# stojicnnnn/3DVision

Measured on AMD Instinct MI355X. Metric: RANSAC hyps/s + ICP iters/s @ 200k-pt clouds, higher is better.
Workload: dtype f32

## Files before the change

3dvision_amd/__init__.py:

```python
import ctypes as C
import os
import sys
import threading
from dataclasses import dataclass, field
from typing import Optional

import numpy as np

_HERE = os.path.dirname(os.path.abspath(__file__))
STUDY_BUILD = os.environ.get("TDV_LIB_VARIANT") == "study"
LIB_PATH = os.path.join(_HERE, "lib3dvision_hip_study.so" if STUDY_BUILD else "lib3dvision_hip.so")

TDV_MASK_THRESHOLD10 = 0
TDV_MASK_NONZERO = 1
TDV_MASK_LABEL_BASE = 256
TDV_VOXEL_ORDER_FIRST = 0
TDV_VOXEL_ORDER_REFERENCE = 1
TIMER_ICP_NN, TIMER_RANSAC_SCORE, TIMER_FEATURE_MATCH, TIMER_KNN, TIMER_RADIUS, TIMER_DEPTH, TIMER_VOXEL, TIMER_FM_INDEX = range(8)
DEPTH_BATCH_MASK_PASSES = 1

ABI_SYMBOLS = [
    "tdv_device_count", "tdv_ctx_create", "tdv_ctx_set_stream", "tdv_ctx_set_icp_search", "tdv_ctx_set_icp_accumulation", "tdv_ctx_last_icp_search", "tdv_ctx_last_batch_lanes", "tdv_ctx_last_voxel_grouping", "tdv_ctx_last_voxel_batch_redone", "tdv_ctx_last_feature_match_path", "tdv_ctx_workspace_bytes", "tdv_ctx_workspace_fill", "tdv_ctx_set_ransac_score", "tdv_ctx_set_ransac_leaf_order", "tdv_ctx_last_ransac_rescore", "tdv_ctx_last_ransac_scored", "tdv_ctx_last_ransac_bound", "tdv_ctx_get_stream", "tdv_ctx_synchronize",
    "tdv_ctx_destroy", "tdv_status_string", "tdv_last_error", "tdv_version", "tdv_timing_enable", "tdv_timing_read",
    "tdv_depth_preprocess", "tdv_deproject", "tdv_depth_to_cloud", "tdv_voxel_downsample", "tdv_estimate_normals",
    "tdv_compute_fpfh", "tdv_feature_match", "tdv_ransac", "tdv_icp", "tdv_icp_correspondences",
    "tdv_icp_dev", "tdv_ransac_dev", "tdv_feature_match_dev", "tdv_estimate_normals_dev", "tdv_compute_fpfh_dev", "tdv_normals_fpfh_dev", "tdv_radix_sort_pairs_dev",
    "tdv_depth_to_cloud_dev", "tdv_voxel_downsample_dev", "tdv_sample_triples", "tdv_sample_triples_batch", "tdv_pose_compose",
    "tdv_register_batch_dev", "tdv_prepare_model_dev", "tdv_bilateral_filter", "tdv_filter_duplicates", "tdv_ransac_score_unit", "tdv_ransac_score_unit_block", "tdv_ransac_score_unit_chunks", "tdv_ransac_batch_size", "tdv_voxel_rules", "tdv_load_ply_ascii", "tdv_load_mask_png", "tdv_load_masks_from_dir",
    "tdv_depth_to_cloud_batch_dev", "tdv_broadcast_model", "tdv_gather_results", "tdv_mask_resize_nearest", "tdv_mask_resize_nearest_dev", "tdv_voxel_downsample_batch_dev", "tdv_voxel_downsample_batch_pinhole_dev",
    "tdv_icp_batch_dev", "tdv_refine_batch_dev", "tdv_ctx_set_icp_loss", "tdv_ctx_get_icp_loss",
    "tdv_gicp", "tdv_gicp_dev", "tdv_gicp_batch_dev",
    "tdv_color_gradients", "tdv_color_gradients_dev", "tdv_colored_icp", "tdv_colored_icp_dev", "tdv_colored_icp_batch_dev",
    "tdv_fgr_default_params", "tdv_fgr", "tdv_fgr_dev", "tdv_fgr_correspondences",
    "tdv_plane_default_params", "tdv_segment_planes", "tdv_segment_planes_dev",
    "tdv_cluster_default_params", "tdv_cluster_dbscan", "tdv_cluster_dbscan_dev",
    "tdv_remove_statistical_outlier", "tdv_remove_statistical_outlier_dev", "tdv_remove_radius_outlier", "tdv_remove_radius_outlier_dev",
    "tdv_iss_default_params", "tdv_iss_keypoints", "tdv_iss_keypoints_dev",
# ... 526 lines not shown
        if kind != "l2" and scale is None:
            raise ValueError("the %s loss needs a scale" % kind)
        _check(self._h, lib().tdv_ctx_set_icp_loss(self._h, self.ICP_LOSS[kind], C.c_float(0.0 if scale is None else float(scale))),
               "tdv_ctx_set_icp_loss")

    def icp_loss(self):
        k = C.c_int(); sc = C.c_float()
        _check(self._h, lib().tdv_ctx_get_icp_loss(self._h, C.byref(k), C.byref(sc)), "tdv_ctx_get_icp_loss")
        return {v: n for n, v in self.ICP_LOSS.items()}[k.value], float(sc.value)

    def set_ransac_score(self, mode):
        _check(self._h, lib().tdv_ctx_set_ransac_score(self._h, {"fast": 0, "exact": 1, "matrix": 2}[mode]), "tdv_ctx_set_ransac_score")

    def set_ransac_leaf_order(self, mode):
        _check(self._h, lib().tdv_ctx_set_ransac_leaf_order(self._h, {"auto": 0, "morton": 1, "classes": 2}[mode]), "tdv_ctx_set_ransac_leaf_order")

    def last_ransac_rescore(self):
        return float(lib().tdv_ctx_last_ransac_rescore(self._h))

    def last_ransac_scored(self):
        return float(lib().tdv_ctx_last_ransac_scored(self._h))

    def last_ransac_bound(self):
        out = (C.c_longlong * 4)()
        lib().tdv_ctx_last_ransac_bound(self._h, out)
        return tuple(int(v) for v in out)

    def last_feature_match_path(self):
        return {0: "none", 1: "scan", 2: "leaf_major", 3: "walk"}[int(lib().tdv_ctx_last_feature_match_path(self._h))]

# ... 1255 lines not shown
```

3dvision_amd/csrc/batch.hip:

```cpp
#include "tdv_internal.hpp"
#include <algorithm>
#include <functional>
#include <thread>
#include <cstdio>
#include <cstdlib>
#include <cstring>
#include <vector>

namespace tdv {

__global__ void k_globalise(const int* __restrict__ local, const int* __restrict__ voff, int n_inst, int total, int* __restrict__ out) {
    const int P = blockIdx.x * blockDim.x + threadIdx.x;
    if (P >= total) return;
    int a = 0, z = n_inst;
    while (z - a > 1) { const int m = (a + z) >> 1; if (voff[m] <= P) a = m; else z = m; }
    out[P] = local[P] + voff[a];
}

__global__ void k_gather_i32(const int* __restrict__ in, const int* __restrict__ idx, int n, int* __restrict__ out) {
    const int p = blockIdx.x * blockDim.x + threadIdx.x;
    if (p < n) out[p] = in[idx[p]];
}

namespace {
// ... 231 lines not shown
    const int L = (int)lane_ctx.size();
    ctx->last_batch_lanes = L;
    auto for_all_instances = [&](const std::function<int(tdv_ctx*, int)>& fn) -> int {
        if (L == 1) {
            int st = TDV_OK;
            for (int b = 0; b < n_instances && st == TDV_OK; ++b) st = fn(ctx, b);
            if (hipStreamSynchronize(ctx->stream) != hipSuccess && st == TDV_OK) st = TDV_ERR_LAUNCH;
            return st;
        }
        TDV_HIP(ctx, hipStreamSynchronize(ctx->stream));
        std::vector<int> status((size_t)L, TDV_OK);
        std::vector<std::thread> workers;
        for (int l = 1; l < L; ++l) {
            tdv_ctx* h = lane_ctx[l];
            h->timing = ctx->timing; h->icp_search = ctx->icp_search; h->icp_accumulate = ctx->icp_accumulate;
            h->icp_loss = ctx->icp_loss; h->icp_loss_scale = ctx->icp_loss_scale; h->ransac_score_mode = ctx->ransac_score_mode; h->ransac_leaf_order = ctx->ransac_leaf_order; h->err[0] = 0;
            workers.emplace_back([&, h, l]() {
                try {
                    if (hipSetDevice(h->device) != hipSuccess) { status[l] = TDV_ERR_NO_DEVICE; return; }
                    status[l] = ws_reset(h);
                    for (int b = l; b < n_instances && status[l] == TDV_OK; b += L) status[l] = fn(h, b);
                    if (hipStreamSynchronize(h->stream) != hipSuccess && status[l] == TDV_OK) status[l] = TDV_ERR_LAUNCH;
                } catch (...) {
                    std::snprintf(h->err, sizeof(h->err), "exception in a helper lane");
                    status[l] = TDV_ERR_INTERNAL;
                }
            });
        }
        try {
            for (int b = 0; b < n_instances && status[0] == TDV_OK; b += L) status[0] = fn(ctx, b);
        } catch (...) {
// ... 255 lines not shown
```

3dvision_amd/csrc/ctx.hip:

```cpp
#include "tdv_internal.hpp"
#include <cmath>
#include <cfloat>
#include <algorithm>
#include <cstring>
#include <vector>

namespace tdv {

int ws_reset(tdv_ctx* ctx) {
    if (ctx->blocks.size() > 1) {
        size_t total = 0;
        TDV_HIP(ctx, hipStreamSynchronize(ctx->stream));
        for (auto& b : ctx->blocks) { total += b.cap; (void)hipFree(b.p); }
        ctx->blocks.clear();
        total = align_up(total + total / 4, (size_t)1 << 20);
        char* p = nullptr;
        TDV_HIP(ctx, hipMalloc((void**)&p, total));
        ctx->blocks.push_back({p, total});
    }
    ctx->cur_block = 0; ctx->cur_off = 0; ctx->used_total = 0;
    return TDV_OK;
}

int ws_alloc_bytes(tdv_ctx* ctx, size_t bytes, void** out) {
// ... 290 lines not shown
    ctx->icp_search = mode;
    return TDV_OK;
}

int tdv_ctx_set_ransac_score(tdv_ctx* ctx, int mode) {
    if (!ctx || (mode != TDV_RANSAC_SCORE_FAST && mode != TDV_RANSAC_SCORE_EXACT && !(tdv::kStudyBuild && mode == TDV_RANSAC_SCORE_MATRIX))) return TDV_ERR_BAD_ARG;
    ctx->ransac_score_mode = mode;
    return TDV_OK;
}

int tdv_ctx_set_ransac_leaf_order(tdv_ctx* ctx, int mode) {
    if (!ctx || mode < TDV_RANSAC_LEAVES_AUTO || mode > TDV_RANSAC_LEAVES_CLASSES) return TDV_ERR_BAD_ARG;
    ctx->ransac_leaf_order = mode;
    return TDV_OK;
}

int tdv_ctx_set_fps_path(tdv_ctx* ctx, int mode) {
    if (!ctx || mode < TDV_FPS_AUTO || mode > TDV_FPS_GRID) return TDV_ERR_BAD_ARG;
    ctx->fps_path = mode;
    return TDV_OK;
}
int tdv_ctx_last_fps_path(tdv_ctx* ctx) { return ctx ? ctx->last_fps_path : 0; }

double tdv_ctx_last_ransac_rescore(tdv_ctx* ctx) { return ctx ? ctx->last_ransac_rescore : -1.0; }

double tdv_ctx_last_ransac_scored(tdv_ctx* ctx) { return ctx ? ctx->last_ransac_scored : 1.0; }
void tdv_ctx_last_ransac_bound(tdv_ctx* ctx, long long out[4]) { if (out) for (int e = 0; e < 4; ++e) out[e] = ctx ? ctx->last_ransac_bound[e] : 0; }

int tdv_ctx_last_icp_search(tdv_ctx* ctx) { return ctx ? ctx->last_icp_search : 0; }
int tdv_ctx_last_feature_match_path(tdv_ctx* ctx) { return ctx ? ctx->last_fm_path : 0; }
// ... 128 lines not shown
```

3dvision_amd/csrc/ransac.hip:

```cpp
#include "tdv_internal.hpp"
#include "host_wait.hpp"
#include "device_linalg.hpp"
#include "ransac_cut.hpp"
#include <cfloat>
#include <climits>
#include <cmath>
#include <cstddef>
#include <cstring>
#include <algorithm>
#include <type_traits>
#include <vector>

namespace tdv {

constexpr float kUnitRoundoff = 5.9604644775390625e-08f;
constexpr float kBandUnit = 16.f * kUnitRoundoff;
constexpr float kBandUnitMatrix = 24.f * kUnitRoundoff;

template <class I>
__device__ __forceinline__ float pair_record(const float* __restrict__ src, const float* __restrict__ tgt, const int* __restrict__ corr, I i, int nt,
                                             int* __restrict__ bad, float4& a, float4& b) {
    int c = corr[i];
    if ((unsigned)c >= (unsigned)nt) { *bad = 1; c = 0; }
    a = make_float4(src[3 * i], src[3 * i + 1], src[3 * i + 2], tgt[3 * c]);
// ... 949 lines not shown
    const unsigned long long m0 = __ballot(far), m1 = __ballot(near), m2 = __ballot(und);
    if (!(m0 | m1 | m2)) return 0;
    int at = 0;
    if (lane < 3) {
        const unsigned long long m = lane == 0 ? m0 : lane == 1 ? m1 : m2;
        int* const n = lane == 0 ? n_live : lane == 1 ? n_near : n_und;
        if (m) at = atomicAdd(n, __popcll(m));
    }
    const unsigned long long below = (1ull << lane) - 1ull;
    const int a0 = __shfl(at, 0, 64) + __popcll(m0 & below), a1 = __shfl(at, 1, 64) + __popcll(m1 & below), a2 = __shfl(at, 2, 64) + __popcll(m2 & below);
    if (far) live[a0] = h;
    if (near) nearl[a1] = h;
    if (und) undl[a2] = h;
    return a2;
}
template <int MODE>
__global__ __launch_bounds__(64 * RB_SPLIT)
void k_ransac_bound(const float* __restrict__ hyp, int h_pad, const TriView triples, int count, const float* __restrict__ leaves, int n_lpairs,
                    const unsigned* __restrict__ pmax, float sqrt_tau, float band_u, const int* __restrict__ state, int ns,
                    int* __restrict__ live, int* __restrict__ n_live, int* __restrict__ und, int* __restrict__ n_und,
                    int* __restrict__ acc, int* __restrict__ ticket, const ListJob lj) {
    const int lane = threadIdx.x & 63, wave = threadIdx.x >> 6;
    const int h = blockIdx.x * 64 + lane;
    __shared__ int s_ub[64];
    if (wave == 0) s_ub[lane] = 0;
    if (MODE == RB_COARSE && threadIdx.x == 0) ticket[blockIdx.x] = 0;
    const bool valid = h < count && triples.valid(h);
    const RbHyp o = rb_load(hyp, h_pad, h, valid, pmax, sqrt_tau, band_u, MODE == RB_COARSE ? 5.f : 3.f);
    const int best = state[0];
    const bool walk = rb_gate(best, ns);
    int fl = 0;
    if (wave == 0 && valid) fl = lj.flags[h];
    const int per = (n_lpairs + RB_SPLIT - 1) / RB_SPLIT, k0 = __builtin_amdgcn_readfirstlane(wave) * per, k1 = min(n_lpairs, k0 + per);
    const int ub = rb_walk(o.r, leaves, k0, k1, o.tb, best, !valid || !o.bounded || !walk);
    __syncthreads();
    if (ub) atomicAdd(&s_ub[lane], ub);
    __syncthreads();
    if (wave != 0) return;
    const int total = s_ub[lane];
    const bool gated = valid && (!o.bounded || !walk);
    const bool close = (fl & RB_CLOSE) != 0;
    const bool undecided = MODE == RB_COARSE && valid && !gated && !close && total > best;
    const bool is_live = gated || close || (MODE == RB_ONE && valid && total > best);
    const bool near = is_live && lj.near && (fl & RB_NEAR);
    const unsigned long long mc = __ballot(close);
    if (mc && lane == 0) atomicAdd(lj.n_close, __popcll(mc));
    const int slot = rb_append3(is_live && !near, near, undecided, lane, h, live, n_live, lj.near, lj.n_near, und, n_und);
    if (MODE == RB_COARSE && undecided) acc[slot] = 0;
}
// ... 132 lines not shown
    int plan[2][8];
    float best12[12];
    double out2[2];
    int sel[4];
    int rec[2][8];
    RansacFar far;
};
constexpr size_t kRansacReadBack = offsetof(RansacBlock, sel);
static_assert(std::is_trivially_copyable<RansacBlock>::value, "memset, copied back");
static_assert(offsetof(RansacBlock, rescored) % 8 == 0 && offsetof(RansacBlock, scored) == offsetof(RansacBlock, rescored) + 8, "the kernels index the two as one u64[2]");
static_assert(offsetof(RansacBlock, out2) % 8 == 0 && offsetof(RansacBlock, out2) + sizeof(double[2]) == kRansacReadBack, "the part read back is a prefix that ends with out2");
struct RansacLive { int n_live[2], n_und[2], n_near[2], n_close[2]; };
static_assert(offsetof(RansacLive, n_und) == offsetof(RansacLive, n_live) + 2 * sizeof(int) && offsetof(RansacLive, n_near) == offsetof(RansacLive, n_live) + 4 * sizeof(int) &&
              offsetof(RansacLive, n_close) == offsetof(RansacLive, n_live) + 6 * sizeof(int), "ransac_plan's n_live[2], n_live[4], n_live[6]");

struct RansacKnobs { bool score_fast, score_mfma, bailout, bound, one_level, leaf_classes, merge, record_copy, upload_inline, order, far, end_event, timer_events; int drop_permille, a_permille, u_cut_permille, fine_y, grown; float far_radius, live_radius; };
static RansacKnobs ransac_knobs(const tdv_ctx* ctx, bool traced, int max_iterations, int ns) {
    RansacKnobs k;
    static const bool score_exact_env = getenv("TDV_RANSAC_SCORE") && !strcmp(getenv("TDV_RANSAC_SCORE"), "exact");
    k.score_fast = !score_exact_env && ctx->ransac_score_mode != TDV_RANSAC_SCORE_EXACT;
    const bool score_mfma_env = study_env("TDV_RANSAC_SCORE") && !strcmp(study_env("TDV_RANSAC_SCORE"), "mfma");
    k.score_mfma = kStudyBuild && k.score_fast && (score_mfma_env || ctx->ransac_score_mode == TDV_RANSAC_SCORE_MATRIX);
    static const bool bailout_env_off = getenv("TDV_RANSAC_BAILOUT") && atoi(getenv("TDV_RANSAC_BAILOUT")) == 0;
    k.bailout = k.score_fast && !k.score_mfma && !traced && !bailout_env_off && max_iterations > 16384;
    k.merge = study_env("TDV_RANSAC_MERGE") && atoi(study_env("TDV_RANSAC_MERGE")) == 1;
    const bool bound_env_off = getenv("TDV_RANSAC_BOUND") && atoi(getenv("TDV_RANSAC_BOUND")) == 0;
    k.bound = k.bailout && !k.merge && !bound_env_off;
    const char* const order_env = getenv("TDV_RANSAC_ORDER");
    k.order = k.bailout && !k.merge && !(order_env && atoi(order_env) == 0);
    k.far = k.order && k.bound && !(order_env && atoi(order_env) == 1);
    k.far_radius = study_env("TDV_RANSAC_FAR_RADIUS") ? (float)atof(study_env("TDV_RANSAC_FAR_RADIUS")) : 4.f;
    k.a_permille = study_env("TDV_RANSAC_FAR_A_PERMILLE") ? atoi(study_env("TDV_RANSAC_FAR_A_PERMILLE")) : 110;
    k.u_cut_permille = study_env("TDV_RANSAC_FAR_UCUT_PERMILLE") ? atoi(study_env("TDV_RANSAC_FAR_UCUT_PERMILLE")) : 22;
    k.live_radius = study_env("TDV_RANSAC_LIVE_RADIUS") ? (float)atof(study_env("TDV_RANSAC_LIVE_RADIUS")) : 20.f;
    k.fine_y = study_env("TDV_RANSAC_FINE_Y") ? std::min(std::max(atoi(study_env("TDV_RANSAC_FINE_Y")), 1), kFineMaxRanges) : 0;
    k.grown = study_env("TDV_RANSAC_GROWN") ? (int)align_up((size_t)std::min(std::max(atoi(study_env("TDV_RANSAC_GROWN")), kRansacBatch), 4 * kRansacBatch), RS_HYP_PER_BLOCK) : kRansacGrown;
    k.leaf_classes = ctx->ransac_leaf_order == TDV_RANSAC_LEAVES_CLASSES || (ctx->ransac_leaf_order == TDV_RANSAC_LEAVES_AUTO && ns >= kRansacLeafClassesMin);
    if (study_env("TDV_RANSAC_LEAF_CLASSES")) k.leaf_classes = atoi(study_env("TDV_RANSAC_LEAF_CLASSES")) == 1;
    k.one_level = study_env("TDV_RANSAC_BOUND_LEVELS") && atoi(study_env("TDV_RANSAC_BOUND_LEVELS")) == 1;
    k.record_copy = study_env("TDV_RANSAC_RECORD") && !strcmp(study_env("TDV_RANSAC_RECORD"), "copy");
    k.end_event = traced || k.record_copy || (study_env("TDV_RANSAC_END") && !strcmp(study_env("TDV_RANSAC_END"), "event"));
    k.timer_events = study_env("TDV_RANSAC_TIMER") && !strcmp(study_env("TDV_RANSAC_TIMER"), "events");
    k.upload_inline = study_env("TDV_RANSAC_UPLOAD") && !strcmp(study_env("TDV_RANSAC_UPLOAD"), "inline");
    k.drop_permille = study_env("TDV_RANSAC_DROP_PERMILLE") ? atoi(study_env("TDV_RANSAC_DROP_PERMILLE")) : 50;
    return k;
}

struct RansacBuf {
    float* hyp; int* counts; void* tri; int* list;
    int *live, *und, *acc, *ticket;
    int *near, *list2, *ubf;
    int* flags;
    int* units;
    int *plan, *rec, *n_live, *n_und, *n_near;
    void* h_tri; int* h_cnt; volatile int* h_rec;
    hipEvent_t ev;
    int seq;
};
struct RansacBatch { int q, cnt, it0; bool bounded; };
struct RangeCut { int per, ranges; };
static RangeCut range_cut(int hb, int n_pchunks) {
    const int per = (n_pchunks + point_ranges(hb, n_pchunks) - 1) / point_ranges(hb, n_pchunks);
    return RangeCut{per, (n_pchunks + per - 1) / per};
}
static int hyp_blocks(int cnt) { return (int)(align_up((size_t)cnt, RS_HYP_PER_BLOCK) / RS_HYP_PER_BLOCK); }
static int score_grid(int hb, int ps) { return 8 * ((hb + 8 / RS_XCD_R - 1) / (8 / RS_XCD_R)) * ((ps + RS_XCD_R - 1) / RS_XCD_R); }
static int unit_grid(int cus) { return std::max(8, (2 * cus + 7) / 8 * 8); }
static int fine_grid(int cus) { return unit_grid(cus); }

struct RansacRun {
    tdv_ctx* ctx; hipStream_t s; RansacKnobs k;
    int ns, nt, max_iterations; float confidence; int* trace;
    float tau, sqrt_tau, band_u;
    int ns_pad, n_pchunks, batch, cap, h_pad, packed, rblocks, n_lpairs = 0, n_cpairs = 0, cus = 0;
    size_t tri_bytes;
    float *pq = nullptr, *pq2 = nullptr, *pq3 = nullptr, *leaves = nullptr, *cleaves = nullptr; double* slabs = nullptr;
    RansacBlock *d = nullptr, *h = nullptr; RansacLive* lv = nullptr;
    unsigned long long* leaf_keys = nullptr; unsigned* leaf_vals = nullptr; bool leaves_built = false;
    unsigned long long* ord_mask = nullptr; int* ord_cnt = nullptr; bool ordered = false;
    unsigned* enc = nullptr;
    RansacBuf buf[2] = {};
    unsigned long long *stamps = nullptr, *h_stamps = nullptr; int n_stamps = 0, stamps_used = 0;
    RansacBatch pending = {}; bool has_pending = false;
    double wave_chunks = 0.0;
    float best_fitness = 0.f; int best_iter = -1, best_inliers = 0, done_iters = 0; bool stop = false;

    TriView tri(const RansacBuf& B) const { return TriView{B.tri, packed}; }
    int setup(const float* d_src, const float* d_tgt, const int* d_corr) {
        ns_pad = (int)align_up((size_t)ns, (size_t)RS_PCH * 64);
        TDV_TRY(ws_alloc(ctx, (size_t)ns_pad * 8, &pq)); TDV_TRY(ws_alloc(ctx, 1, &d));
        TDV_HIP(ctx, hipMemsetAsync(d, 0, sizeof(RansacBlock), s));
        k_gather_pq<<<(ns_pad + 255) / 256, 256, 0, s>>>(d_src, d_tgt, d_corr, ns, ns_pad, nt, pq, &d->bad, &d->pmax);
        if (k.bound) TDV_TRY(leaf_alloc());
#ifdef TDV_STUDY
        if (k.score_mfma) TDV_TRY(mfma_pack(ctx, pq, ns, ns_pad, &pq3));
        else
// ... 21 lines not shown
                TDV_TRY(ws_alloc(ctx, (size_t)h_pad, &B.acc)); TDV_TRY(ws_alloc(ctx, (size_t)h_pad / 64, &B.ticket));
                TDV_TRY(ws_alloc(ctx, (size_t)h_pad, &B.flags));
            }
            TDV_TRY(ws_alloc(ctx, 1, &lv));
        }
        if (k.far) for (RansacBuf& B : buf) { TDV_TRY(ws_alloc(ctx, (size_t)h_pad, &B.near)); TDV_TRY(ws_alloc(ctx, (size_t)h_pad, &B.list2)); TDV_TRY(ws_alloc(ctx, (size_t)h_pad, &B.ubf)); }
        rblocks = (ns + 255) / 256; TDV_TRY(ws_alloc(ctx, (size_t)2 * rblocks, &slabs));
        if (ctx->timing && k.score_fast && !k.score_mfma && !k.timer_events) {
            n_stamps = 2 * n_batches + 1;
            TDV_TRY(ws_alloc(ctx, (size_t)2 * n_stamps, &stamps));
            TDV_HIP(ctx, hipMemsetAsync(stamps, 0xff, (size_t)n_stamps * 8, s));
            TDV_HIP(ctx, hipMemsetAsync(stamps + n_stamps, 0, (size_t)n_stamps * 8, s));
        }
        const size_t sz_blk = align_up(sizeof(RansacBlock), 64), sz_tri = align_up((size_t)cap * tri_bytes, 64), sz_cnt = trace ? align_up((size_t)cap * 4, 64) : 0;
        const size_t sz_grown = k.bailout ? 2 * align_up((size_t)k.grown * 16, 64) : 0;
        TDV_TRY(pin_reserve(ctx, sz_blk + std::max(2 * sz_tri, sz_grown) + 2 * sz_cnt + (size_t)n_stamps * 16));
        h = reinterpret_cast<RansacBlock*>(ctx->pin); h->bad = 0;
        h->rec[0][4] = h->rec[1][4] = 0;
        h_stamps = reinterpret_cast<unsigned long long*>(ctx->pin + sz_blk + 2 * sz_tri + 2 * sz_cnt);
        if (trace) TDV_HIP(ctx, hipMemcpyAsync(&h->bad, &d->bad, 4, hipMemcpyDeviceToHost, s));
        for (int q = 0; q < 2; ++q) {
            RansacBuf& B = buf[q];
            B.plan = d->plan[q]; B.rec = d->rec[q]; B.n_live = lv ? &lv->n_live[q] : nullptr; B.n_und = lv ? &lv->n_und[q] : nullptr; B.n_near = lv ? &lv->n_near[q] : nullptr;
            B.h_tri = ctx->pin + sz_blk + q * sz_tri; B.h_cnt = reinterpret_cast<int*>(ctx->pin + sz_blk + 2 * sz_tri + q * sz_cnt); B.h_rec = h->rec[q];
        }
        if (k.end_event) {
            buf[0].ev = event_acquire(ctx); buf[1].ev = event_acquire(ctx);
            if (!buf[0].ev || !buf[1].ev) { release_events(); return TDV_ERR_OOM; }
        }
        return TDV_OK;
    }
    ScoreStamp next_stamp() { if (!stamps || stamps_used >= n_stamps) return ScoreStamp{nullptr, nullptr}; const int e = stamps_used++; return ScoreStamp{stamps + e, stamps + n_stamps + e}; }
    int score_slot() const { return stamps ? -1 : TDV_TIMER_RANSAC_SCORE; }
    void launch_score(int grid, const ScoreJob& a, const ScoreJob& b, int g1) {
        const ScoreStamp st = next_stamp();
        if (st.t0) k_ransac_score_fast<true><<<grid, RS_BLOCK, 0, s>>>(a, b, g1, h_pad, pq2, n_pchunks, tau, &d->rescored, st);
        else k_ransac_score_fast<false><<<grid, RS_BLOCK, 0, s>>>(a, b, g1, h_pad, pq2, n_pchunks, tau, &d->rescored, st);
    }
    int batch_size(int it0) const { return k.bailout ? ransac_batch_size(it0, k.grown) : batch; }
// ... 10 lines not shown
    }
    int leaf_build() {
        const int n_leaves = (ns + RL_LEAF - 1) / RL_LEAF;
        unsigned long long* const keys = leaf_keys; unsigned* const vals = leaf_vals;
        TDV_HIP(ctx, hipMemsetAsync(leaves, 0, (size_t)n_lpairs * 32 * sizeof(float), s));
        TDV_HIP(ctx, hipMemsetAsync(cleaves, 0, (size_t)n_cpairs * 32 * sizeof(float), s));
        TDV_HIP(ctx, hipMemsetAsync(enc, 0xff, 24, s)); TDV_HIP(ctx, hipMemsetAsync(enc + 6, 0, 24, s));
        k_leaf_bounds<<<(ns + 255) / 256, 256, 0, s>>>(pq, ns, enc);
        k_leaf_keys<<<(ns + 255) / 256, 256, 0, s>>>(pq, ns, enc, k.leaf_classes && ordered ? ord_mask : nullptr, keys, vals);
        TDV_TRY(radix_sort_pairs_dev(ctx, keys, keys + ns, vals, vals + ns, (size_t)ns, RL_CLASS_BIT + (k.leaf_classes ? 1 : 0)));
        k_leaf_build<<<(n_leaves * RL_LEAF + 255) / 256, 256, 0, s>>>(pq, ns, vals + ns, leaves, cleaves);
        leaves_built = true;
        TDV_CHECK_LAUNCH(ctx); return TDV_OK;
    }

    int draw(TripleStream& idx, int q, int it0) {
        const int cnt = std::min(batch_size(it0), max_iterations - it0);
        if (packed) idx.next_batch_packed(cnt, static_cast<uint64_t*>(buf[q].h_tri));
        else idx.next_batch(cnt, static_cast<int*>(buf[q].h_tri));
        return cnt;
    }
    int hypotheses(const RansacBatch& b) {
        const RansacBuf& B = buf[b.q];
        if (k.upload_inline) TDV_HIP(ctx, hipMemcpyAsync(B.tri, B.h_tri, (size_t)b.cnt * tri_bytes, hipMemcpyHostToDevice, s));
        const PlanJob plan{d->state, k.bailout ? B.plan : nullptr, ns, n_pchunks, k.drop_permille, b.bounded ? B.n_live : nullptr, B.units, k.bailout ? unit_words(b.cnt) : 0,
                           k.far && b.bounded ? &d->far : nullptr, k.a_permille};
        const PreJob pre{b.bounded ? B.flags : nullptr, B.ubf, k.far ? &d->far : nullptr, enc, d->best12, k.live_radius, k.u_cut_permille};
        k_ransac_hypotheses<<<(slots(b.cnt) + 255) / 256, 256, 0, s>>>(pq, tri(B), k.upload_inline ? nullptr : B.h_tri, b.cnt, slots(b.cnt), h_pad, B.hyp, &d->pmax, sqrt_tau, B.counts, band_u, plan, pre);
        return TDV_OK;
    }
    int score_all(const RansacBatch& b) {
        const RansacBuf& B = buf[b.q]; const int hb = hyp_blocks(b.cnt);
        ScopedTimer tm(ctx, k.score_fast && !k.score_mfma ? score_slot() : TDV_TIMER_RANSAC_SCORE);
#ifdef TDV_STUDY
        if (k.score_mfma) wave_chunks += mfma_score(s, B.hyp, h_pad, pq3, ns, b.cnt, tau, B.counts, &d->rescored);
        else
#endif
        if (k.score_fast) {
            const ScoreJob ja{B.hyp, B.counts, nullptr, nullptr, hb, range_cut(hb, n_pchunks).ranges, nullptr, nullptr, nullptr};
            const int gA = score_grid(hb, ja.ps);
            launch_score(gA, ja, ja, gA);
            wave_chunks += (double)hb * (RS_BLOCK / 64) * (double)n_pchunks;
        } else {
            const RangeCut c = range_cut(h_pad / RS_HYP_PER_BLOCK, n_pchunks);
            k_ransac_score<<<dim3(hb, c.ranges), RS_BLOCK, 0, s>>>(B.hyp, h_pad, pq2, n_pchunks, c.per, tau, B.counts);
        }
        return TDV_OK;
    }
    void bound(const RansacBatch& b) {
        const RansacBuf& B = buf[b.q]; const int bgrid = (b.cnt + 63) / 64;
        const ListJob lj{B.flags, k.far ? B.near : nullptr, B.n_near, B.n_live + 6};
        if (k.one_level)
            k_ransac_bound<RB_ONE><<<bgrid, 64 * RB_SPLIT, 0, s>>>(B.hyp, h_pad, tri(B), b.cnt, leaves, n_lpairs, &d->pmax, sqrt_tau, band_u,
                                                                   d->state, ns, B.live, B.n_live, nullptr, nullptr, nullptr, nullptr, lj);
        else {
            k_ransac_bound<RB_COARSE><<<bgrid, 64 * RB_SPLIT, 0, s>>>(B.hyp, h_pad, tri(B), b.cnt, cleaves, n_cpairs, &d->pmax, sqrt_tau, band_u,
                                                                      d->state, ns, B.live, B.n_live, B.und, B.n_und, B.acc, B.ticket, lj);
            const FineJob fj{B.hyp, leaves, &d->pmax, d->state, B.und, B.n_und, B.live, B.n_live, B.acc, B.ticket, lj, h_pad, n_lpairs, k.fine_y, sqrt_tau, band_u};
            k_ransac_bound_fine<<<fine_grid(cus), 64 * RB_SPLIT, 0, s>>>(fj);
        }
    }
    void point_order() {
        RansacFar* const far = k.far ? &d->far : nullptr;
        k_order_flags<<<order_blocks(), RO_BLOCK, 0, s>>>(pq, ns, d->state, d->best12, tau, ord_mask, ord_cnt, far, std::max(tau, k.far_radius * k.far_radius * tau));
        k_order_scatter<<<order_blocks(), RO_BLOCK, 0, s>>>(pq, ns, ord_mask, ord_cnt, pq2, far);
        ordered = true;
    }
    ScoreJob job_a(const RansacBatch& b) const { return ScoreJob{buf[b.q].hyp, buf[b.q].counts, buf[b.q].plan, nullptr, hyp_blocks(b.cnt), range_cut(hyp_blocks(b.cnt), n_pchunks).ranges, nullptr, nullptr, nullptr}; }
    void phase1(const RansacBatch& b) {
        const RansacBuf& B = buf[b.q];
        const int hbw = slots(b.cnt) / RS_BLOCK;
        const ScoreJob ja = job_a(b), jl{B.hyp, B.counts, B.plan, B.live, hbw, 0, B.n_live, B.units, nullptr};
// ... 54 lines not shown
        std::snprintf(ctx->err, sizeof(ctx->err), "ransac: the stream ran dry and batch %d's record never came", B.seq);
        return TDV_ERR_LAUNCH;
    }
    int enqueue_merged(const RansacBatch& b) {
        if (has_pending) {
            const ScoreJob ja = job_a(b);
            TDV_TRY(phase2(pending, &ja, score_grid(ja.hb, ja.ps)));
            TDV_TRY(finish(pending, true));
        } else phase1(b);
        TDV_TRY(select(b));
        pending = b; has_pending = true;
        return TDV_OK;
    }
    int finish_pending() { has_pending = false; TDV_TRY(phase2(pending)); return finish(pending, true); }

    int enqueue(int q, int cnt, int it0) {
        const RansacBatch b{q, cnt, it0, k.bound && it0 != 0};
        if (k.order && it0 != 0 && !ordered) point_order();
        if (b.bounded && !leaves_built) TDV_TRY(leaf_build());
        TDV_TRY(hypotheses(b));
        if (!k.bailout) { TDV_TRY(score_all(b)); return finish(b, false); }
        if (k.merge) return enqueue_merged(b);
        if (b.bounded) bound(b);
        phase1(b);
        TDV_TRY(select(b));
        TDV_TRY(phase2(b));
        return finish(b, true);
    }

    void consume_record(const RansacBuf& B, int it0, int cnt) {
        const int k_best = B.h_rec[0], k_stop = B.h_rec[2];
        if (k_best >= 0) {
            best_inliers = B.h_rec[1]; best_iter = it0 + k_best;
            best_fitness = static_cast<float>(best_inliers) / static_cast<float>((size_t)ns);
        }
        stop = k_stop >= 0; done_iters = it0 + (stop ? k_stop + 1 : cnt);
    }
    int consume_trace(const RansacBuf& B, int it0, int cnt) {
        const TriView t{B.h_tri, packed};
        int batch_best = -1;
        for (int j = 0; j < cnt; ++j) {
            done_iters = it0 + j + 1;
            if (!t.valid(j)) { trace[it0 + j] = -1; continue; }
            const int inl = trace[it0 + j] = B.h_cnt[j];
            const float fitness = static_cast<float>(inl) / static_cast<float>((size_t)ns);
            if (fitness > best_fitness) { best_fitness = fitness; best_iter = it0 + j; best_inliers = inl; batch_best = j; }
            if (fitness > confidence) { stop = true; break; }
        }
        if (batch_best >= 0)
            TDV_HIP(ctx, hipMemcpy2DAsync(d->best12, 4, B.hyp + batch_best, (size_t)h_pad * 4, 4, 12, hipMemcpyDeviceToDevice, s));
        return TDV_OK;
    }
    int loop(uint32_t seed) {
        TripleStream idx(seed, (uint64_t)ns);
        int cur = 0, it0 = 0, cnt_cur = draw(idx, cur, it0);
        TDV_TRY(enqueue(cur, cnt_cur, 0));
        while (cnt_cur > 0 && !stop) {
            const int nxt = cur ^ 1, it_next = it0 + cnt_cur; int cnt_next = 0;
            if (it_next < max_iterations) {
                cnt_next = draw(idx, nxt, it_next);
                TDV_TRY(enqueue(nxt, cnt_next, it_next));
            } else if (has_pending) TDV_TRY(finish_pending());
            const RansacBuf& B = buf[cur];
            TDV_TRY(wait_batch(B));
            if (trace ? h->bad : B.h_rec[3]) { std::snprintf(ctx->err, sizeof(ctx->err), "ransac: a correspondence index lies outside [0, %d)", nt); return TDV_ERR_BAD_ARG; }
            if (trace) TDV_TRY(consume_trace(B, it0, cnt_cur));
            else consume_record(B, it0, cnt_cur);
            cur = nxt; it0 = it_next; cnt_cur = cnt_next;
        }
        return TDV_OK;
    }

    int read_stamps() {
        if (!ctx->wall_clock_khz) TDV_HIP(ctx, hipDeviceGetAttribute(&ctx->wall_clock_khz, hipDeviceAttributeWallClockRate, ctx->device));
        unsigned long long ticks = 0ull;
        for (int e = 0; e < stamps_used; ++e) if (h_stamps[n_stamps + e] > h_stamps[e]) ticks += h_stamps[n_stamps + e] - h_stamps[e];
        TimerSlot& t = ctx->timers[TDV_TIMER_RANSAC_SCORE];
        if (ctx->wall_clock_khz > 0) t.total_ms += (double)ticks / (double)ctx->wall_clock_khz;
        t.launches += stamps_used;
        return TDV_OK;
    }

    int result(tdv_ransac_result* out) {
// ... 37 lines not shown
    if (ns == 0 || nt == 0 || max_iterations == 0) return TDV_OK;
    int* d_match = nullptr;
    if (!d_corr_in) { TDV_TRY(ws_alloc(ctx, (size_t)ns, &d_match)); TDV_TRY(feature_match_dev(ctx, d_fs, ns, d_ft, nt, d_match)); }
    const int* d_corr = d_corr_in ? d_corr_in : d_match;
    RansacRun r;
    r.ctx = ctx; r.s = ctx->stream; r.k = ransac_knobs(ctx, trace_inliers != nullptr, max_iterations, ns);
    r.ns = ns; r.nt = nt; r.max_iterations = max_iterations; r.confidence = confidence; r.trace = trace_inliers;
    r.tau = tau_lt(voxel * 1.5f);
    r.sqrt_tau = std::nextafter((float)std::sqrt((double)r.tau), INFINITY);
    r.band_u = r.k.score_mfma ? kBandUnitMatrix : kBandUnit;
    TDV_TRY(r.setup(d_src, d_tgt, d_corr));
    const int status = r.loop(seed);
    (void)hipStreamSynchronize(r.s);
    ctx->last_ransac_rescore = -1.0; ctx->last_ransac_scored = 1.0;
    for (long long& v : ctx->last_ransac_bound) v = 0;
    r.release_events();
    return status != TDV_OK ? status : r.result(out);
}


struct RbResult { float T[12]; int best_iter, inliers, iterations_run, pad; };

__global__ __launch_bounds__(1024)
void k_rb_sample(const unsigned* __restrict__ raw, int n_raw, const int* __restrict__ off, int H, int* __restrict__ idx_out , int* __restrict__ fail) {
    const int b = blockIdx.x, n = off[b + 1] - off[b];
    if (n <= 0) return;
    const unsigned range = (unsigned)n, thr = (0u - range) % range;
    int* out = idx_out + (size_t)b * 3 * H;
    __shared__ int s_wave[16];
    __shared__ int s_produced;
// ... 195 lines not shown
```

3dvision_amd/csrc/tdv_internal.hpp:

```cpp
#pragma once
#include <hip/hip_runtime.h>
#include <climits>
#include <cmath>
#include <cstdint>
#include <cstdio>
#include <cstdlib>
#include <cstring>
#include <vector>
#include "tdv_hip.h"
#include "depth_frames.hpp"

namespace tdv {

struct TimerSlot {
    double total_ms = 0.0;
    int launches = 0;
    std::vector<std::pair<hipEvent_t, hipEvent_t>> pending;
};

}

struct tdv_ctx {
    int device = 0;
    hipStream_t stream = nullptr;
    bool own_stream = false;
    struct Block { char* p; size_t cap; };
    std::vector<Block> blocks;
    size_t cur_block = 0, cur_off = 0, high_water = 0, used_total = 0;
    char* pin = nullptr;
    size_t pin_cap = 0;
    char err[512] = {0};
    bool timing = false;
    int icp_search = 0;
    int icp_accumulate = 0;
    int icp_loss = 0;
    float icp_loss_scale = 0.f;
    int ransac_leaf_order = 0;
    int ransac_score_mode = 0;
    double last_ransac_rescore = -1.0;
    long long last_ransac_bound[4] = {0, 0, 0, 0};
    double last_ransac_scored = 1.0;
    int last_voxel_grouping = 0;
    int last_voxel_batch_redone = -1;
    int last_fm_path = 0;
    int last_batch_lanes = 0;
    int fps_path = 0;
    int last_fps_path = 0;
    int icp_launches = 0;
    int last_icp_launches = 0;
    int icp_probe_cache = 0;
    int last_icp_probe_misses = -1;
    int last_icp_search = 0;
// ... 247 lines not shown
```

include/tdv_hip.h:

```cpp
#ifndef TDV_HIP_H
#define TDV_HIP_H

#include <stddef.h>
#include <stdint.h>

#ifdef __cplusplus
extern "C" {
#endif

typedef struct tdv_ctx tdv_ctx;

typedef enum tdv_status {
    TDV_OK = 0,
    TDV_ERR_NO_DEVICE = -1,
    TDV_ERR_BAD_ARG = -2,
    TDV_ERR_OOM = -3,
    TDV_ERR_LAUNCH = -4,
    TDV_ERR_INTERNAL = -5
} tdv_status;

int tdv_device_count(int* count);
int tdv_ctx_create(int device, tdv_ctx** out);
int tdv_ctx_set_stream(tdv_ctx* ctx, void* hip_stream);
void* tdv_ctx_get_stream(tdv_ctx* ctx);
// ... 19 lines not shown
int tdv_ctx_last_icp_probe_misses(tdv_ctx* ctx);
#define TDV_ICP_LOSS_L2 0
#define TDV_ICP_LOSS_HUBER 1
#define TDV_ICP_LOSS_TUKEY 2
#define TDV_ICP_LOSS_CAUCHY 3
int tdv_ctx_set_icp_loss(tdv_ctx* ctx, int loss, float scale);
int tdv_ctx_get_icp_loss(tdv_ctx* ctx, int* loss, float* scale);
#define TDV_RANSAC_SCORE_FAST 0
#define TDV_RANSAC_SCORE_EXACT 1
#define TDV_RANSAC_SCORE_MATRIX 2
int tdv_ctx_set_ransac_score(tdv_ctx* ctx, int mode);
#define TDV_RANSAC_LEAVES_AUTO 0
#define TDV_RANSAC_LEAVES_MORTON 1
#define TDV_RANSAC_LEAVES_CLASSES 2
int tdv_ctx_set_ransac_leaf_order(tdv_ctx* ctx, int mode);
double tdv_ctx_last_ransac_rescore(tdv_ctx* ctx);
double tdv_ctx_last_ransac_scored(tdv_ctx* ctx);
int tdv_ctx_last_icp_search(tdv_ctx* ctx);
#define TDV_FM_PATH_SCAN 1
#define TDV_FM_PATH_LEAF_MAJOR 2
#define TDV_FM_PATH_WALK 3
int tdv_ctx_last_feature_match_path(tdv_ctx* ctx);
#define TDV_VOXEL_GROUPING_TABLE 1
#define TDV_VOXEL_GROUPING_PIXELS 2
int tdv_ctx_last_voxel_grouping(tdv_ctx* ctx);
int tdv_ctx_last_voxel_batch_redone(tdv_ctx* ctx);
int tdv_ctx_last_batch_lanes(tdv_ctx* ctx);
unsigned long long tdv_ctx_workspace_bytes(tdv_ctx* ctx);
int tdv_ctx_workspace_fill(tdv_ctx* ctx, int byte);
const char* tdv_status_string(int status);
// ... 554 lines not shown
```

Measured before the change: 9507.

## Stage next batch's triples into device memory during RANSAC bound kernel

Adds a staged triple-upload path. The host draws the next batch's sampled triples one batch ahead into a third pinned slot, and the coarse bound kernel copies them into the other buffer's device triple array while it runs. The next hypotheses kernel then reads the triples from device memory instead of across the bus from pinned host memory. This hides the host-to-device transfer latency inside an existing kernel, at the cost of extra global traffic in the bound kernel and more complex slot bookkeeping.

```diff
diff --git a/3dvision_amd/__init__.py b/3dvision_amd/__init__.py
--- a/3dvision_amd/__init__.py
+++ b/3dvision_amd/__init__.py
@@ -20,7 +20,7 @@
 DEPTH_BATCH_MASK_PASSES = 1
 
 ABI_SYMBOLS = [
-    "tdv_device_count", "tdv_ctx_create", "tdv_ctx_set_stream", "tdv_ctx_set_icp_search", "tdv_ctx_set_icp_accumulation", "tdv_ctx_last_icp_search", "tdv_ctx_last_batch_lanes", "tdv_ctx_last_voxel_grouping", "tdv_ctx_last_voxel_batch_redone", "tdv_ctx_last_feature_match_path", "tdv_ctx_workspace_bytes", "tdv_ctx_workspace_fill", "tdv_ctx_set_ransac_score", "tdv_ctx_set_ransac_leaf_order", "tdv_ctx_last_ransac_rescore", "tdv_ctx_last_ransac_scored", "tdv_ctx_last_ransac_bound", "tdv_ctx_get_stream", "tdv_ctx_synchronize",
+    "tdv_device_count", "tdv_ctx_create", "tdv_ctx_set_stream", "tdv_ctx_set_icp_search", "tdv_ctx_set_icp_accumulation", "tdv_ctx_last_icp_search", "tdv_ctx_last_batch_lanes", "tdv_ctx_last_voxel_grouping", "tdv_ctx_last_voxel_batch_redone", "tdv_ctx_last_feature_match_path", "tdv_ctx_workspace_bytes", "tdv_ctx_workspace_fill", "tdv_ctx_set_ransac_score", "tdv_ctx_set_ransac_leaf_order", "tdv_ctx_set_ransac_triples", "tdv_ctx_last_ransac_staged", "tdv_ctx_last_ransac_rescore", "tdv_ctx_last_ransac_scored", "tdv_ctx_last_ransac_bound", "tdv_ctx_get_stream", "tdv_ctx_synchronize",
     "tdv_ctx_destroy", "tdv_status_string", "tdv_last_error", "tdv_version", "tdv_timing_enable", "tdv_timing_read",
     "tdv_depth_preprocess", "tdv_deproject", "tdv_depth_to_cloud", "tdv_voxel_downsample", "tdv_estimate_normals",
     "tdv_compute_fpfh", "tdv_feature_match", "tdv_ransac", "tdv_icp", "tdv_icp_correspondences",
@@ -577,6 +577,12 @@
 
     def set_ransac_leaf_order(self, mode):
         _check(self._h, lib().tdv_ctx_set_ransac_leaf_order(self._h, {"auto": 0, "morton": 1, "classes": 2}[mode]), "tdv_ctx_set_ransac_leaf_order")
+
+    def set_ransac_triples(self, mode):
+        _check(self._h, lib().tdv_ctx_set_ransac_triples(self._h, {"auto": 0, "direct": 1, "staged": 2}[mode]), "tdv_ctx_set_ransac_triples")
+
+    def last_ransac_staged(self):
+        return int(lib().tdv_ctx_last_ransac_staged(self._h))
 
     def last_ransac_rescore(self):
         return float(lib().tdv_ctx_last_ransac_rescore(self._h))
diff --git a/3dvision_amd/csrc/batch.hip b/3dvision_amd/csrc/batch.hip
--- a/3dvision_amd/csrc/batch.hip
+++ b/3dvision_amd/csrc/batch.hip
@@ -269,7 +269,7 @@
         for (int l = 1; l < L; ++l) {
             tdv_ctx* h = lane_ctx[l];
             h->timing = ctx->timing; h->icp_search = ctx->icp_search; h->icp_accumulate = ctx->icp_accumulate;
-            h->icp_loss = ctx->icp_loss; h->icp_loss_scale = ctx->icp_loss_scale; h->ransac_score_mode = ctx->ransac_score_mode; h->ransac_leaf_order = ctx->ransac_leaf_order; h->err[0] = 0;
+            h->icp_loss = ctx->icp_loss; h->icp_loss_scale = ctx->icp_loss_scale; h->ransac_score_mode = ctx->ransac_score_mode; h->ransac_leaf_order = ctx->ransac_leaf_order; h->ransac_triples = ctx->ransac_triples; h->err[0] = 0;
             workers.emplace_back([&, h, l]() {
                 try {
                     if (hipSetDevice(h->device) != hipSuccess) { status[l] = TDV_ERR_NO_DEVICE; return; }
diff --git a/3dvision_amd/csrc/ctx.hip b/3dvision_amd/csrc/ctx.hip
--- a/3dvision_amd/csrc/ctx.hip
+++ b/3dvision_amd/csrc/ctx.hip
@@ -328,6 +328,13 @@
     ctx->ransac_leaf_order = mode;
     return TDV_OK;
 }
+
+int tdv_ctx_set_ransac_triples(tdv_ctx* ctx, int mode) {
+    if (!ctx || mode < TDV_RANSAC_TRIPLES_AUTO || mode > TDV_RANSAC_TRIPLES_STAGED) return TDV_ERR_BAD_ARG;
+    ctx->ransac_triples = mode;
+    return TDV_OK;
+}
+int tdv_ctx_last_ransac_staged(tdv_ctx* ctx) { return ctx ? ctx->last_ransac_staged : 0; }
 
 int tdv_ctx_set_fps_path(tdv_ctx* ctx, int mode) {
     if (!ctx || mode < TDV_FPS_AUTO || mode > TDV_FPS_GRID) return TDV_ERR_BAD_ARG;
diff --git a/3dvision_amd/csrc/ransac.hip b/3dvision_amd/csrc/ransac.hip
--- a/3dvision_amd/csrc/ransac.hip
+++ b/3dvision_amd/csrc/ransac.hip
@@ -987,12 +987,13 @@
     if (und) undl[a2] = h;
     return a2;
 }
-template <int MODE>
+struct StageJob { const uint64_t* src; uint64_t* dst; int cnt; };
+template <int MODE, bool STAGE = false>
 __global__ __launch_bounds__(64 * RB_SPLIT)
 void k_ransac_bound(const float* __restrict__ hyp, int h_pad, const TriView triples, int count, const float* __restrict__ leaves, int n_lpairs,
                     const unsigned* __restrict__ pmax, float sqrt_tau, float band_u, const int* __restrict__ state, int ns,
                     int* __restrict__ live, int* __restrict__ n_live, int* __restrict__ und, int* __restrict__ n_und,
-                    int* __restrict__ acc, int* __restrict__ ticket, const ListJob lj) {
+                    int* __restrict__ acc, int* __restrict__ ticket, const ListJob lj, const StageJob stage) {
     const int lane = threadIdx.x & 63, wave = threadIdx.x >> 6;
     const int h = blockIdx.x * 64 + lane;
     __shared__ int s_ub[64];
@@ -1004,8 +1005,16 @@
     const bool walk = rb_gate(best, ns);
     int fl = 0;
     if (wave == 0 && valid) fl = lj.flags[h];
+    const int gid = blockIdx.x * blockDim.x + threadIdx.x;
+    uint64_t sw = 0;
+    if (STAGE) sw = stage.src[min(gid, stage.cnt - 1)];
     const int per = (n_lpairs + RB_SPLIT - 1) / RB_SPLIT, k0 = __builtin_amdgcn_readfirstlane(wave) * per, k1 = min(n_lpairs, k0 + per);
     const int ub = rb_walk(o.r, leaves, k0, k1, o.tb, best, !valid || !o.bounded || !walk);
+    if (STAGE) {
+        if (gid < stage.cnt) stage.dst[gid] = sw;
+        const int all = gridDim.x * blockDim.x;
+        for (int i = gid + all; i < stage.cnt; i += all) stage.dst[i] = stage.src[i];
+    }
     __syncthreads();
     if (ub) atomicAdd(&s_ub[lane], ub);
     __syncthreads();
@@ -1168,7 +1177,7 @@
 static_assert(offsetof(RansacLive, n_und) == offsetof(RansacLive, n_live) + 2 * sizeof(int) && offsetof(RansacLive, n_near) == offsetof(RansacLive, n_live) + 4 * sizeof(int) &&
               offsetof(RansacLive, n_close) == offsetof(RansacLive, n_live) + 6 * sizeof(int), "ransac_plan's n_live[2], n_live[4], n_live[6]");
 
-struct RansacKnobs { bool score_fast, score_mfma, bailout, bound, one_level, leaf_classes, merge, record_copy, upload_inline, order, far, end_event, timer_events; int drop_permille, a_permille, u_cut_permille, fine_y, grown; float far_radius, live_radius; };
+struct RansacKnobs { bool score_fast, score_mfma, bailout, bound, one_level, leaf_classes, merge, record_copy, upload_inline, order, far, end_event, timer_events; int drop_permille, a_permille, u_cut_permille, fine_y, grown, triples; float far_radius, live_radius; };
 static RansacKnobs ransac_knobs(const tdv_ctx* ctx, bool traced, int max_iterations, int ns) {
     RansacKnobs k;
     static const bool score_exact_env = getenv("TDV_RANSAC_SCORE") && !strcmp(getenv("TDV_RANSAC_SCORE"), "exact");
@@ -1196,6 +1205,9 @@
     k.end_event = traced || k.record_copy || (study_env("TDV_RANSAC_END") && !strcmp(study_env("TDV_RANSAC_END"), "event"));
     k.timer_events = study_env("TDV_RANSAC_TIMER") && !strcmp(study_env("TDV_RANSAC_TIMER"), "events");
     k.upload_inline = study_env("TDV_RANSAC_UPLOAD") && !strcmp(study_env("TDV_RANSAC_UPLOAD"), "inline");
+    k.triples = ctx->ransac_triples;
+    if (study_env("TDV_RANSAC_UPLOAD") && !strcmp(study_env("TDV_RANSAC_UPLOAD"), "staged")) k.triples = TDV_RANSAC_TRIPLES_STAGED;
+    if (study_env("TDV_RANSAC_UPLOAD") && !strcmp(study_env("TDV_RANSAC_UPLOAD"), "direct")) k.triples = TDV_RANSAC_TRIPLES_DIRECT;
     k.drop_permille = study_env("TDV_RANSAC_DROP_PERMILLE") ? atoi(study_env("TDV_RANSAC_DROP_PERMILLE")) : 50;
     return k;
 }
@@ -1208,10 +1220,12 @@
     int* units;
     int *plan, *rec, *n_live, *n_und, *n_near;
     void* h_tri; int* h_cnt; volatile int* h_rec;
+    bool staged;
     hipEvent_t ev;
     int seq;
 };
-struct RansacBatch { int q, cnt, it0; bool bounded; };
+struct RansacBatch { int q, cnt, it0; bool bounded, staged; };
+struct RansacDrawn { int it0, cnt, slot; };
 struct RangeCut { int per, ranges; };
 static RangeCut range_cut(int hb, int n_pchunks) {
     const int per = (n_pchunks + point_ranges(hb, n_pchunks) - 1) / point_ranges(hb, n_pchunks);
@@ -1234,6 +1248,9 @@
     unsigned long long* ord_mask = nullptr; int* ord_cnt = nullptr; bool ordered = false;
     unsigned* enc = nullptr;
     RansacBuf buf[2] = {};
+    char* h_slots = nullptr; size_t sz_slot = 0; int n_slots = 2; bool stage = false;
+    int n_drawn = 0, it_drawn = 0, n_staged = 0;
+    void* slot_ptr(int slot) const { return h_slots + (size_t)slot * sz_slot; }
     unsigned long long *stamps = nullptr, *h_stamps = nullptr; int n_stamps = 0, stamps_used = 0;
     RansacBatch pending = {}; bool has_pending = false;
     double wave_chunks = 0.0;
@@ -1285,15 +1302,18 @@
         }
         const size_t sz_blk = align_up(sizeof(RansacBlock), 64), sz_tri = align_up((size_t)cap * tri_bytes, 64), sz_cnt = trace ? align_up((size_t)cap * 4, 64) : 0;
         const size_t sz_grown = k.bailout ? 2 * align_up((size_t)k.grown * 16, 64) : 0;
-        TDV_TRY(pin_reserve(ctx, sz_blk + std::max(2 * sz_tri, sz_grown) + 2 * sz_cnt + (size_t)n_stamps * 16));
+        const size_t tri_room = std::max(2 * sz_tri, sz_grown);
+        TDV_TRY(pin_reserve(ctx, sz_blk + tri_room + 2 * sz_cnt + (size_t)n_stamps * 16));
+        stage = k.triples != TDV_RANSAC_TRIPLES_DIRECT && k.bound && !k.one_level && !k.upload_inline && !trace && packed && 3 * sz_tri <= tri_room;
+        n_slots = stage ? 3 : 2; sz_slot = sz_tri; h_slots = ctx->pin + sz_blk;
         h = reinterpret_cast<RansacBlock*>(ctx->pin); h->bad = 0;
         h->rec[0][4] = h->rec[1][4] = 0;
-        h_stamps = reinterpret_cast<unsigned long long*>(ctx->pin + sz_blk + 2 * sz_tri + 2 * sz_cnt);
+        h_stamps = reinterpret_cast<unsigned long long*>(ctx->pin + sz_blk + tri_room + 2 * sz_cnt);
         if (trace) TDV_HIP(ctx, hipMemcpyAsync(&h->bad, &d->bad, 4, hipMemcpyDeviceToHost, s));
         for (int q = 0; q < 2; ++q) {
             RansacBuf& B = buf[q];
             B.plan = d->plan[q]; B.rec = d->rec[q]; B.n_live = lv ? &lv->n_live[q] : nullptr; B.n_und = lv ? &lv->n_und[q] : nullptr; B.n_near = lv ? &lv->n_near[q] : nullptr;
-            B.h_tri = ctx->pin + sz_blk + q * sz_tri; B.h_cnt = reinterpret_cast<int*>(ctx->pin + sz_blk + 2 * sz_tri + q * sz_cnt); B.h_rec = h->rec[q];
+            B.h_tri = slot_ptr(q); B.staged = false; B.h_cnt = reinterpret_cast<int*>(ctx->pin + sz_blk + 2 * sz_tri + q * sz_cnt); B.h_rec = h->rec[q];
         }
         if (k.end_event) {
             buf[0].ev = event_acquire(ctx); buf[1].ev = event_acquire(ctx);
@@ -1334,11 +1354,12 @@
         TDV_CHECK_LAUNCH(ctx); return TDV_OK;
     }
 
-    int draw(TripleStream& idx, int q, int it0) {
-        const int cnt = std::min(batch_size(it0), max_iterations - it0);
-        if (packed) idx.next_batch_packed(cnt, static_cast<uint64_t*>(buf[q].h_tri));
-        else idx.next_batch(cnt, static_cast<int*>(buf[q].h_tri));
-        return cnt;
+    RansacDrawn draw(TripleStream& idx) {
+        const RansacDrawn dn{it_drawn, std::min(batch_size(it_drawn), max_iterations - it_drawn), n_drawn % n_slots};
+        if (packed) idx.next_batch_packed(dn.cnt, static_cast<uint64_t*>(slot_ptr(dn.slot)));
+        else idx.next_batch(dn.cnt, static_cast<int*>(slot_ptr(dn.slot)));
+        ++n_drawn; it_drawn += dn.cnt;
+        return dn;
     }
     int hypotheses(const RansacBatch& b) {
         const RansacBuf& B = buf[b.q];
@@ -1346,7 +1367,7 @@
         const PlanJob plan{d->state, k.bailout ? B.plan : nullptr, ns, n_pchunks, k.drop_permille, b.bounded ? B.n_live : nullptr, B.units, k.bailout ? unit_words(b.cnt) : 0,
                            k.far && b.bounded ? &d->far : nullptr, k.a_permille};
         const PreJob pre{b.bounded ? B.flags : nullptr, B.ubf, k.far ? &d->far : nullptr, enc, d->best12, k.live_radius, k.u_cut_permille};
-        k_ransac_hypotheses<<<(slots(b.cnt) + 255) / 256, 256, 0, s>>>(pq, tri(B), k.upload_inline ? nullptr : B.h_tri, b.cnt, slots(b.cnt), h_pad, B.hyp, &d->pmax, sqrt_tau, B.counts, band_u, plan, pre);
+        k_ransac_hypotheses<<<(slots(b.cnt) + 255) / 256, 256, 0, s>>>(pq, tri(B), k.upload_inline || b.staged ? nullptr : B.h_tri, b.cnt, slots(b.cnt), h_pad, B.hyp, &d->pmax, sqrt_tau, B.counts, band_u, plan, pre);
         return TDV_OK;
     }
     int score_all(const RansacBatch& b) {
@@ -1367,15 +1388,17 @@
         }
         return TDV_OK;
     }
-    void bound(const RansacBatch& b) {
+    void bound(const RansacBatch& b, const RansacDrawn* next) {
         const RansacBuf& B = buf[b.q]; const int bgrid = (b.cnt + 63) / 64;
         const ListJob lj{B.flags, k.far ? B.near : nullptr, B.n_near, B.n_live + 6};
         if (k.one_level)
             k_ransac_bound<RB_ONE><<<bgrid, 64 * RB_SPLIT, 0, s>>>(B.hyp, h_pad, tri(B), b.cnt, leaves, n_lpairs, &d->pmax, sqrt_tau, band_u,
-                                                                   d->state, ns, B.live, B.n_live, nullptr, nullptr, nullptr, nullptr, lj);
+                                                                   d->state, ns, B.live, B.n_live, nullptr, nullptr, nullptr, nullptr, lj, StageJob{nullptr, nullptr, 0});
         else {
-            k_ransac_bound<RB_COARSE><<<bgrid, 64 * RB_SPLIT, 0, s>>>(B.hyp, h_pad, tri(B), b.cnt, cleaves, n_cpairs, &d->pmax, sqrt_tau, band_u,
-                                                                      d->state, ns, B.live, B.n_live, B.und, B.n_und, B.acc, B.ticket, lj);
+            const StageJob sj = next ? StageJob{static_cast<const uint64_t*>(slot_ptr(next->slot)), static_cast<uint64_t*>(buf[b.q ^ 1].tri), next->cnt} : StageJob{nullptr, nullptr, 0};
+            const auto kernel = next && next->cnt > 0 ? k_ransac_bound<RB_COARSE, true> : k_ransac_bound<RB_COARSE, false>;
+            kernel<<<bgrid, 64 * RB_SPLIT, 0, s>>>(B.hyp, h_pad, tri(B), b.cnt, cleaves, n_cpairs, &d->pmax, sqrt_tau, band_u,
+                                                   d->state, ns, B.live, B.n_live, B.und, B.n_und, B.acc, B.ticket, lj, sj);
             const FineJob fj{B.hyp, leaves, &d->pmax, d->state, B.und, B.n_und, B.live, B.n_live, B.acc, B.ticket, lj, h_pad, n_lpairs, k.fine_y, sqrt_tau, band_u};
             k_ransac_bound_fine<<<fine_grid(cus), 64 * RB_SPLIT, 0, s>>>(fj);
         }
@@ -1460,14 +1483,16 @@
     }
     int finish_pending() { has_pending = false; TDV_TRY(phase2(pending)); return finish(pending, true); }
 
-    int enqueue(int q, int cnt, int it0) {
-        const RansacBatch b{q, cnt, it0, k.bound && it0 != 0};
+    int enqueue(int q, const RansacDrawn& dn, bool staged, const RansacDrawn* next) {
+        const int cnt = dn.cnt, it0 = dn.it0;
+        buf[q].h_tri = slot_ptr(dn.slot); buf[q].staged = staged;
+        const RansacBatch b{q, cnt, it0, k.bound && it0 != 0, staged};
         if (k.order && it0 != 0 && !ordered) point_order();
         if (b.bounded && !leaves_built) TDV_TRY(leaf_build());
         TDV_TRY(hypotheses(b));
         if (!k.bailout) { TDV_TRY(score_all(b)); return finish(b, false); }
         if (k.merge) return enqueue_merged(b);
-        if (b.bounded) bound(b);
+        if (b.bounded) bound(b, next);
         phase1(b);
         TDV_TRY(select(b));
         TDV_TRY(phase2(b));
@@ -1497,22 +1522,30 @@
             TDV_HIP(ctx, hipMemcpy2DAsync(d->best12, 4, B.hyp + batch_best, (size_t)h_pad * 4, 4, 12, hipMemcpyDeviceToDevice, s));
         return TDV_OK;
     }
+    int enqueue_next(TripleStream& idx, int q, const RansacDrawn& dn, bool staged, RansacDrawn& ahead, bool& has_ahead) {
+        has_ahead = stage && k.bound && dn.it0 != 0 && dn.it0 + dn.cnt < max_iterations;
+        if (has_ahead) ahead = draw(idx);
+        return enqueue(q, dn, staged, has_ahead ? &ahead : nullptr);
+    }
     int loop(uint32_t seed) {
         TripleStream idx(seed, (uint64_t)ns);
-        int cur = 0, it0 = 0, cnt_cur = draw(idx, cur, it0);
-        TDV_TRY(enqueue(cur, cnt_cur, 0));
-        while (cnt_cur > 0 && !stop) {
-            const int nxt = cur ^ 1, it_next = it0 + cnt_cur; int cnt_next = 0;
+        int cur = 0;
+        RansacDrawn dc = draw(idx), ahead = {}; bool has_ahead = false;
+        TDV_TRY(enqueue_next(idx, cur, dc, false, ahead, has_ahead));
+        while (dc.cnt > 0 && !stop) {
+            const int nxt = cur ^ 1, it_next = dc.it0 + dc.cnt; RansacDrawn dn = {it_next, 0, 0};
             if (it_next < max_iterations) {
-                cnt_next = draw(idx, nxt, it_next);
-                TDV_TRY(enqueue(nxt, cnt_next, it_next));
+                const bool staged = has_ahead;
+                dn = staged ? ahead : draw(idx);
+                TDV_TRY(enqueue_next(idx, nxt, dn, staged, ahead, has_ahead));
             } else if (has_pending) TDV_TRY(finish_pending());
             const RansacBuf& B = buf[cur];
             TDV_TRY(wait_batch(B));
             if (trace ? h->bad : B.h_rec[3]) { std::snprintf(ctx->err, sizeof(ctx->err), "ransac: a correspondence index lies outside [0, %d)", nt); return TDV_ERR_BAD_ARG; }
-            if (trace) TDV_TRY(consume_trace(B, it0, cnt_cur));
-            else consume_record(B, it0, cnt_cur);
-            cur = nxt; it0 = it_next; cnt_cur = cnt_next;
+            if (trace) TDV_TRY(consume_trace(B, dc.it0, dc.cnt));
+            else consume_record(B, dc.it0, dc.cnt);
+            n_staged += B.staged ? 1 : 0;
+            cur = nxt; dc = dn;
         }
         return TDV_OK;
     }
@@ -1580,6 +1613,7 @@
     (void)hipStreamSynchronize(r.s);
     ctx->last_ransac_rescore = -1.0; ctx->last_ransac_scored = 1.0;
     for (long long& v : ctx->last_ransac_bound) v = 0;
+    ctx->last_ransac_staged = r.n_staged;
     r.release_events();
     return status != TDV_OK ? status : r.result(out);
 }
diff --git a/3dvision_amd/csrc/tdv_internal.hpp b/3dvision_amd/csrc/tdv_internal.hpp
--- a/3dvision_amd/csrc/tdv_internal.hpp
+++ b/3dvision_amd/csrc/tdv_internal.hpp
@@ -36,6 +36,8 @@
     int icp_loss = 0;
     float icp_loss_scale = 0.f;
     int ransac_leaf_order = 0;
+    int ransac_triples = 0;
+    int last_ransac_staged = 0;
     int ransac_score_mode = 0;
     double last_ransac_rescore = -1.0;
     long long last_ransac_bound[4] = {0, 0, 0, 0};
diff --git a/include/tdv_hip.h b/include/tdv_hip.h
--- a/include/tdv_hip.h
+++ b/include/tdv_hip.h
@@ -57,6 +57,11 @@
 #define TDV_RANSAC_LEAVES_MORTON 1
 #define TDV_RANSAC_LEAVES_CLASSES 2
 int tdv_ctx_set_ransac_leaf_order(tdv_ctx* ctx, int mode);
+#define TDV_RANSAC_TRIPLES_AUTO 0
+#define TDV_RANSAC_TRIPLES_DIRECT 1
+#define TDV_RANSAC_TRIPLES_STAGED 2
+int tdv_ctx_set_ransac_triples(tdv_ctx* ctx, int mode);
+int tdv_ctx_last_ransac_staged(tdv_ctx* ctx);
 double tdv_ctx_last_ransac_rescore(tdv_ctx* ctx);
 double tdv_ctx_last_ransac_scored(tdv_ctx* ctx);
 int tdv_ctx_last_icp_search(tdv_ctx* ctx);
```

After: 9750 (median of 6 runs). 2.6% higher.
